# votnhan/VN_celeb_face_recognition

Hardware: AMD Instinct MI355X
Metric: embeddings/sec @ bs=256 (InceptionResnetV1, 160x160) (higher is better)
Workload: dtype bf16

## Files before the change

### vn_celeb_face_recognition_amd/csrc/autotune.cpp

```cpp
#include "engine.h"

#include <algorithm>
#include <cstdio>
#include <cstdlib>
#include <map>

namespace vnf {

EncoderEnv EncoderEnv::read() {
  auto env_int = [](const char* name, int dflt) { const char* v = getenv(name); return v ? atoi(v) : dflt; };
  EncoderEnv e;
  e.fuse = env_int("VNF_FUSE", e.fuse);
  e.direct_stem = env_int("VNF_DIRECT_STEM", e.direct_stem);
  e.stem1a_mfma = env_int("VNF_STEM1A_MFMA", e.stem1a_mfma);
  e.stem_chunk = env_int("VNF_STEM_CHUNK", e.stem_chunk);
  e.ir100_chunk1 = env_int("VNF_IR100_CHUNK1", e.ir100_chunk1);
  e.ir100_chunk2 = env_int("VNF_IR100_CHUNK2", e.ir100_chunk2);
  e.retina_fuse = env_int("VNF_RETINA_FUSE", e.retina_fuse);
  e.ws_persist = env_int("VNF_WS_PERSIST", e.ws_persist);
  e.autotune = env_int("VNF_AUTOTUNE", e.autotune);
  e.force_cfg = env_int("VNF_FORCE_CFG", e.force_cfg);
  e.tune_lanes = env_int("VNF_TUNE_LANES", e.tune_lanes);
  e.autotune_log = env_int("VNF_AUTOTUNE_LOG", e.autotune_log);
  e.tune_final = env_int("VNF_TUNE_FINAL", 1) != 0;
  if (const char* cache = getenv("VNF_TUNE_CACHE")) e.tune_cache = cache;
  return e;
}

int Encoder::autotune() {
  const int enabled = env.autotune, force = env.force_cfg;
  if (!enabled && force < -1) return VNF_OK;
  std::map<std::string, int> cache;
  const char* cache_path = env.tune_cache.empty() ? nullptr : env.tune_cache.c_str();
  bool cache_dirty = false;
  if (cache_path && enabled) {
    if (FILE* f = fopen(cache_path, "r")) {
      char key[256];
      int c;
      while (fscanf(f, "%255s %d", key, &c) == 2) cache[key] = c;
      fclose(f);
    }
  }
  VNF_HIP(hipDeviceSynchronize());
  struct Timers {
    hipEvent_t e0 = nullptr, e1 = nullptr;
    hipStream_t lane_s[4] = {nullptr, nullptr, nullptr, nullptr};
    hipEvent_t lane_e[4] = {nullptr, nullptr, nullptr, nullptr};
    ~Timers() {
      if (e0) (void)hipEventDestroy(e0);
      if (e1) (void)hipEventDestroy(e1);
      for (int l = 0; l < 4; ++l) {
        if (lane_e[l]) (void)hipEventDestroy(lane_e[l]);
// ... 113 lines not shown
```

### vn_celeb_face_recognition_amd/csrc/conv_device.h

```cpp
#pragma once
#include <atomic>

#include "kernels.h"
#include "split_f16.h"

namespace vnf {

typedef __bf16 bf16x8_t __attribute__((ext_vector_type(8)));
typedef _Float16 f16x8_t __attribute__((ext_vector_type(8)));
typedef float f32x4_t __attribute__((ext_vector_type(4)));

struct KArgs {
  const char* x;
  const char* w;
  const float* bias;
  const int4* ktab;
  const char* res;
  const float* slope;
  const char* zero;
  int ldx, H, W, Ho, Wo, sh, sw, ph, pw;
  int K, Kpad, nkt;
  int wrs, wts;
  int ncls, cout_pad;
  int M, Cout, tiles_n, nblk;
// ... 374 lines not shown
          char* const dptr = a.seg_ptr[sg];
          if (a.out_f32)
            store8<float>(dptr + ((size_t)m * a.seg_ld[sg] + (c - a.seg_c0[sg])) * 4, v);
          else
            store8<T>(dptr + ((size_t)m * a.seg_ld[sg] + (c - a.seg_c0[sg])) * ES, v);
        }
      }
      __syncthreads();
    }
  }
}

__device__ __forceinline__ void glds16(const void* gsrc, unsigned lds_base) {
  unsigned keep;
  asm volatile(
      "s_mov_b32 %0, m0\n\ts_mov_b32 m0, %2\n\ts_nop 0\n\tglobal_load_lds_dwordx4 %1, off\n\ts_mov_b32 m0, %0"
      : "=&s"(keep)
      : "v"(gsrc), "s"(lds_base)
      : "memory");
}

template <int N>
__device__ __forceinline__ void wait_dma_and_barrier() {
  asm volatile("s_waitcnt vmcnt(%0) lgkmcnt(0)\n\ts_barrier" ::"n"(N) : "memory");
}

constexpr int patch_epi_bytes(int bm, int bn, int wm) {
  return bm * (bn + 4) * 4 <= 64 * 1024 ? bm * (bn + 4) * 4 : (bm / wm) * (bn + 4) * 4;
}
int patch_num_cfgs();
bool patch_cfg_ok(const ConvArgs& a, int pcfg);
bool patch_cfg_tile(int pcfg, ConvTile& t);
hipError_t launch_patch(const ConvArgs& a, const KArgs& k, int pcfg, hipStream_t s);

int ws_num_cfgs();
bool ws_cfg_ok(const ConvArgs& a, int wcfg);
bool ws_cfg_tile(int wcfg, ConvTile& t);
hipError_t launch_ws(const ConvArgs& a, const KArgs& k, int wcfg, hipStream_t s);

}
```

### vn_celeb_face_recognition_amd/csrc/conv_igemm.hip

```cpp
#include <mutex>
#include <type_traits>
#include <utility>

#include "block35.h"
#include "conv_device.h"

namespace vnf {

template <int AP, int RS>
__device__ __forceinline__ void row_setup(const KArgs& a, int m0, int lrow, int (&abase)[AP], int (&ahi)[AP],
                                          int (&awi)[AP]) {
  const int HoWo = a.Ho * a.Wo;
#pragma unroll
  for (int p = 0; p < AP; ++p) {
    const int m = m0 + lrow + RS * p;
    if (m < a.M) {
      const int n = m / HoWo, r = m - n * HoWo;
      const int ho = r / a.Wo, wo = r - ho * a.Wo;
      ahi[p] = ho * a.sh - a.ph;
      awi[p] = wo * a.sw - a.pw;
      abase[p] = ((n * a.H + ahi[p]) * a.W + awi[p]) * a.ldx;
    } else {
      ahi[p] = -(1 << 24);
      awi[p] = 0;
// ... 264 lines not shown
}

static bool dma_capable(const ConvArgs& a) { return (a.Kpad / (128 / dtype_size(a.dtype))) * 8 * 16 <= 24 * 1024; }

bool conv_cfg_ok(const ConvArgs& a, int cfg) {
  if (cfg >= kNumCfgs + patch_num_cfgs()) return dma_capable(a) && ws_cfg_ok(a, cfg - kNumCfgs - patch_num_cfgs());
  if (cfg >= kNumCfgs) return dma_capable(a) && patch_cfg_ok(a, cfg - kNumCfgs);
  if (cfg < 0) return false;
  const TileCfg& c = kCfgs[cfg];
  if (c.bn > 32 && a.Cout <= c.bn / 2) return false;
  if (((a.Cout + c.bn - 1) / c.bn) * c.bn > a.cout_pad) return false;
  if ((c.bn % 64) && a.Cout % c.bn) return false;
  const int lds = c.s * (c.bm + c.bn) * 128;
  return lds <= 160 * 1024;
}

template <typename T, size_t... I>
static hipError_t launch_cfg(int cfg, const KArgs& k, hipStream_t s, std::index_sequence<I...>) {
  static constexpr hipError_t (*kLaunch[])(const KArgs&, hipStream_t) = {
      launch_dma<T, kCfgs[I].bm, kCfgs[I].bn, kCfgs[I].wm, kCfgs[I].wn, kCfgs[I].s>...};
  return (unsigned)cfg < sizeof...(I) ? kLaunch[cfg](k, s) : hipErrorInvalidValue;
}
template <typename T>
static hipError_t launch_cfg(int cfg, const KArgs& k, hipStream_t s) {
  return launch_cfg<T>(cfg, k, s, std::make_index_sequence<kNumCfgs>{});
}

template <typename T>
static hipError_t launch_typed(const ConvArgs& a, const KArgs& k, hipStream_t s) {
  if (!k.zero) return hipErrorOutOfMemory;
  if (a.cfg >= kNumCfgs + patch_num_cfgs() && conv_cfg_ok(a, a.cfg)) return launch_ws(a, k, a.cfg - kNumCfgs - patch_num_cfgs(), s);
  if (a.cfg >= kNumCfgs && conv_cfg_ok(a, a.cfg)) return launch_patch(a, k, a.cfg - kNumCfgs, s);
  if (a.cfg >= 0 && conv_cfg_ok(a, a.cfg)) return launch_cfg<T>(a.cfg, k, s);
  auto fits = [&](int) { return true; };
  int bn = 128;
  while (bn > 32 && !(fits(bn) && (a.Cout % bn == 0 || a.Cout > 2 * bn))) bn >>= 1;
  if (!fits(bn)) return hipErrorInvalidValue;
  auto blocks = [&](int bm_, int bn_) { return ((a.M + bm_ - 1) / bm_) * ((a.Cout + bn_ - 1) / bn_); };
  while (bn > 64 && blocks(128, bn) < 512) bn >>= 1;
  int bm = 128;
  if (bn <= 64 && blocks(128, bn) < 512) bm = 64;
  const int id = bm == 128 ? (bn == 128 ? 0 : bn == 64 ? 1 : 2) : (bn == 64 ? 3 : 4);
  return launch_cfg<T>(id, k, s);
}

hipError_t launch_conv(const ConvArgs& a, hipStream_t s) {
  if (a.M <= 0) return hipSuccess;
  const int es = dtype_size(a.dtype);
  const int bke = 128 / es;
  if (a.Cout % 8 || a.Kpad % bke || a.nseg < 1 || a.nseg > 4) return hipErrorInvalidValue;
  KArgs k;
  k.x = (const char*)a.x; k.w = (const char*)a.w; k.bias = a.bias; k.ktab = a.ktab;
  k.res = (const char*)a.res; k.slope = a.slope; k.zero = zero_page();
  k.ldx = a.ldx; k.H = a.H; k.W = a.W; k.Ho = a.Ho; k.Wo = a.Wo;
  k.sh = a.sh; k.sw = a.sw; k.ph = a.ph; k.pw = a.pw;
  k.K = a.K; k.Kpad = a.Kpad; k.nkt = a.Kpad / bke;
  k.wrs = a.Kpad * es; k.wts = 128;
  k.ncls = a.ncls; k.cout_pad = a.cout_pad;
  k.M = a.M; k.Cout = a.Cout; k.tiles_n = 0; k.nblk = 0;
  k.ldres = a.ldres; k.act = a.act; k.out_f32 = a.out_f32;
  k.nseg = a.nseg;
  k.KH = a.KH; k.KW = a.KW; k.Cin = a.Cin; k.pp = k.Wp = k.Hv = k.patch_bytes = k.lds_bytes = 0; k.dbg = nullptr;
  for (int i = 0; i < 4; ++i) {
    k.seg_c0[i] = i < a.nseg ? a.seg[i].c0 : 1 << 30;
    k.seg_c1[i] = i < a.nseg ? a.seg[i].c1 : 1 << 30;
    k.seg_ld[i] = i < a.nseg ? a.seg[i].ld : 0;
// ... 14 lines not shown
```

### vn_celeb_face_recognition_amd/csrc/conv_patch.hip

```cpp
#include <map>
#include <mutex>
#include <tuple>
#include <type_traits>
#include <utility>

#include "conv_device.h"
#include "stamp.h"

namespace vnf {

template <typename T, int BM, int BN, int WM, int WN, int S, bool DBG = false>
__global__ __launch_bounds__(WM* WN * 64) void conv_patch_kernel(const KArgs a) {
  extern __shared__ __attribute__((aligned(16))) char smem[];
  constexpr int ES = (int)sizeof(T);
  constexpr int CH = 16 / ES, BKE = 128 / ES;
  constexpr int WTM = BM / WM, WTN = BN / WN, TM = WTM / 16, TN = WTN / 16;
  constexpr int NW = WM * WN, NT = NW * 64, RS = NT / 8;
  constexpr int BPM = (BN + RS - 1) / RS;
  constexpr int STAGE = BN * 128;
  constexpr int EPI = patch_epi_bytes(BM, BN, WM);
  static_assert((NW == 4 || NW == 8) && S >= 3 && BPM <= 8, "4 or 8 waves, ring of >= 3 stages");

  const int tid = threadIdx.x, lane = tid & 63;
  const int wave = __builtin_amdgcn_readfirstlane(tid >> 6);
// ... 172 lines not shown
#pragma unroll
      for (int i = 0; i < TM; ++i)
#pragma unroll
        for (int j = 0; j < TN; ++j) mma_cross(acc[i][j], wh[0][j], wf[1][j], xh[0][i], xf[1][i]);
    } else {
#pragma unroll
      for (int i = 0; i < TM; ++i)
#pragma unroll
        for (int j = 0; j < TN; ++j) mma_cross(acc[i][j], wh[1][j], wf[1][j], xh[1][i], xf[1][i]);
    }
  } else {
    bool pend = false;
    for (int kt = 0; kt < nkt; ++kt) {
      stamp();
      sync_tile(kt);
      stamp();
      read_frags(kt, 0, t0);
      if (pend) mma(1);
      pend = BKE / 2 < a.K - kt * BKE;
      if (pend) read_frags(kt, 1, t1);
      t0 = sP[(kt + 1) * 8 + fgrp];
      t1 = sP[(kt + 1) * 8 + 4 + fgrp];
      mma(0);
    }
    if (pend) mma(1);
  }
  stamp();
  __syncthreads();
  stamp();
  conv_epilogue<T, BM, BN, WM, WN, EPI>(a, acc, smem, m0, n0, a.lds_bytes);
  stamp();
}

struct PatchCfg { int bm, bn, wm, wn, s; };
static constexpr PatchCfg kPatch[] = {
    {256, 32, 8, 1, 3},  {256, 32, 4, 1, 3},  {128, 32, 4, 1, 3},  {256, 64, 4, 2, 3},  {128, 64, 4, 2, 3},
    {128, 64, 2, 2, 3},  {64, 64, 2, 2, 4},   {256, 192, 4, 2, 3}, {128, 192, 2, 4, 3}, {64, 192, 2, 4, 3},
    {128, 256, 2, 4, 3}, {256, 256, 4, 2, 3}, {128, 128, 2, 4, 3}, {256, 128, 4, 2, 3}, {64, 128, 2, 4, 3},
    {64, 128, 2, 2, 4},
    {256, 64, 4, 2, 6},  {128, 64, 4, 2, 6},  {256, 128, 4, 2, 4}, {256, 32, 8, 1, 6},
    {128, 96, 4, 1, 3},  {128, 96, 2, 2, 3},  {64, 192, 1, 4, 3},
    {192, 192, 4, 2, 3},
};
constexpr int kNumPatch = (int)(sizeof(kPatch) / sizeof(kPatch[0]));

int patch_num_cfgs() { return kNumPatch; }
bool patch_cfg_tile(int pcfg, ConvTile& t) {
  if (pcfg < 0 || pcfg >= kNumPatch) return false;
  t = ConvTile{1, kPatch[pcfg].bm, kPatch[pcfg].bn, kPatch[pcfg].wm, kPatch[pcfg].wn, kPatch[pcfg].s};
  return true;
}

static int patch_rows_max(int Wo, int Ho, int KH, int BM) {
  static std::mutex mu;
  static std::map<std::tuple<int, int, int, int>, int> cache;
  std::lock_guard<std::mutex> lk(mu);
  const auto key = std::make_tuple(Wo, Ho, KH, BM);
  auto it = cache.find(key);
  if (it != cache.end()) return it->second;
  int best = 0;
  const long long HoWo = (long long)Ho * Wo;
  for (long long t = 0; t <= HoWo; ++t) {
    const long long m0 = t * BM, m1 = m0 + BM - 1;
    const long long g0 = m0 / Wo, g1 = m1 / Wo;
    const long long v0 = g0 + (g0 / Ho) * (KH - 1), v1 = g1 + (g1 / Ho) * (KH - 1) + KH - 1;
    if (v1 - v0 + 1 > best) best = (int)(v1 - v0 + 1);
  }
  cache[key] = best;
  return best;
}

struct PatchGeom { int pp, Wp, Hv, patch_bytes, lds; };

static bool patch_geom(const ConvArgs& a, const PatchCfg& c, PatchGeom& g) {
  const int es = dtype_size(a.dtype), ch = dtype_chan_align(a.dtype);
  const int planes = a.dtype == F16P ? 2 : 1;
  if (a.sh != 1 || a.sw != 1 || a.Cin % ch || a.Ho != a.H + 2 * a.ph - a.KH + 1 || a.Wo != a.W + 2 * a.pw - a.KW + 1)
    return false;
  g.pp = a.Cin / ch;
  while (g.pp % 4 != 2) ++g.pp;
  g.Wp = a.W + 2 * a.pw;
  g.Hv = a.H + 2 * a.ph;
  const long long slots = (long long)patch_rows_max(a.Wo, a.Ho, a.KH, c.bm) * g.Wp * g.pp;
  if (slots * 16 * planes > 160 * 1024) return false;
  g.patch_bytes = (int)((slots * 16 + 1023) / 1024 * 1024) * planes;
  const int nkt = a.Kpad / (128 / es);
  int lds = c.s * c.bn * 128 + (((nkt + 1) * 8 * 4 + 15) & ~15) + 16 + g.patch_bytes;
  const int epi = patch_epi_bytes(c.bm, c.bn, c.wm);
  if (lds < epi) lds = epi;
  g.lds = lds;
  return lds <= 160 * 1024;
}

bool patch_cfg_ok(const ConvArgs& a, int pcfg) {
  if (pcfg < 0 || pcfg >= kNumPatch) return false;
  const PatchCfg& c = kPatch[pcfg];
  if (a.KH * a.KW == 1) return false;
  if (c.bn > 32 && a.Cout <= c.bn / 2) return false;
  if (((a.Cout + c.bn - 1) / c.bn) * c.bn > a.cout_pad) return false;
  if ((c.bn % 64) && a.Cout % c.bn) return false;
  PatchGeom g;
  return patch_geom(a, c, g);
}

template <typename T, int BM, int BN, int WM, int WN, int S>
static hipError_t launch_one(const KArgs& k, int lds, hipStream_t s) {
  allow_dynamic_lds<conv_patch_kernel<T, BM, BN, WM, WN, S>>(160 * 1024);
  KArgs kk = k;
  const int tiles_m = (k.M + BM - 1) / BM;
  kk.tiles_n = (k.Cout + BN - 1) / BN;
  kk.nblk = tiles_m * kk.tiles_n;
  hipLaunchKernelGGL((conv_patch_kernel<T, BM, BN, WM, WN, S>), dim3(kk.nblk), dim3(WM * WN * 64), lds, s, kk);
  return hipGetLastError();
}

template <typename T, size_t... I>
static hipError_t launch_patch_typed(int pcfg, const KArgs& k, int lds, hipStream_t s, std::index_sequence<I...>) {
  static constexpr hipError_t (*kLaunch[])(const KArgs&, int, hipStream_t) = {
      launch_one<T, kPatch[I].bm, kPatch[I].bn, kPatch[I].wm, kPatch[I].wn, kPatch[I].s>...};
  return (unsigned)pcfg < sizeof...(I) ? kLaunch[pcfg](k, lds, s) : hipErrorInvalidValue;
}
template <typename T>
static hipError_t launch_patch_typed(int pcfg, const KArgs& k, int lds, hipStream_t s) {
  return launch_patch_typed<T>(pcfg, k, lds, s, std::make_index_sequence<kNumPatch>{});
}

#ifdef VNF_STAMPS
constexpr PatchCfg kStamp = {256, 192, 4, 2, 3};
constexpr int patch_cfg_id(const PatchCfg& q) {
  for (int i = 0; i < kNumPatch; ++i)
    if (kPatch[i].bm == q.bm && kPatch[i].bn == q.bn && kPatch[i].wm == q.wm && kPatch[i].wn == q.wn && kPatch[i].s == q.s) return i;
  return -1;
}
constexpr int kStampId = patch_cfg_id(kStamp);
static_assert(kStampId >= 0, "the instrumented tile is one of kPatch");

static hipError_t launch_patch_stamped(const KArgs& k, int lds, hipStream_t s) {
  constexpr auto kernel = conv_patch_kernel<__bf16, kStamp.bm, kStamp.bn, kStamp.wm, kStamp.wn, kStamp.s, true>;
  KArgs kk = k;
  kk.tiles_n = (k.Cout + kStamp.bn - 1) / kStamp.bn;
  kk.nblk = ((k.M + kStamp.bm - 1) / kStamp.bm) * kk.tiles_n;
  return stamped_launch(
      "VNF_PATCH_STAMP", 8 * 40, s,
      [&](long long* dbuf) {
        kk.dbg = dbuf;
        allow_dynamic_lds<kernel>(160 * 1024);
        hipLaunchKernelGGL(kernel, dim3(kk.nblk), dim3(kStamp.wm * kStamp.wn * 64), lds, s, kk);
      },
      [&](FILE* f, const long long* host) {
        fprintf(f, "launch M=%d N=%d nkt=%d nblk=%d\n", k.M, k.Cout, k.nkt, kk.nblk);
        for (int w = 0; w < 8; ++w) {
          fprintf(f, "%d", w);
          for (int i = 0; i < 40; ++i) fprintf(f, " %lld", host[w * 40 + i] ? host[w * 40 + i] - host[0] : -1LL);
          fprintf(f, "\n");
        }
      });
}
#endif

hipError_t launch_patch(const ConvArgs& a, const KArgs& k, int pcfg, hipStream_t s) {
  if (!patch_cfg_ok(a, pcfg) || !k.zero) return hipErrorInvalidValue;
  PatchGeom g;
  patch_geom(a, kPatch[pcfg], g);
  KArgs kk = k;
  kk.KH = a.KH; kk.KW = a.KW; kk.Cin = a.Cin;
  kk.pp = g.pp; kk.Wp = g.Wp; kk.Hv = g.Hv; kk.patch_bytes = g.patch_bytes; kk.lds_bytes = g.lds;
#ifdef VNF_STAMPS
  if (getenv("VNF_PATCH_STAMP") && pcfg == kStampId && a.dtype == BF16 &&
      ((k.M + kStamp.bm - 1) / kStamp.bm) * ((k.Cout + kStamp.bn - 1) / kStamp.bn) > 700)
    return launch_patch_stamped(kk, g.lds, s);
#endif
  switch (a.dtype) {
    case BF16: return launch_patch_typed<__bf16>(pcfg, kk, g.lds, s);
    case F16: return launch_patch_typed<_Float16>(pcfg, kk, g.lds, s);
    case F32: return launch_patch_typed<float>(pcfg, kk, g.lds, s);
    case F16X2: return launch_patch_typed<sf16>(pcfg, kk, g.lds, s);
    case F16P: return launch_patch_typed<pf16>(pcfg, kk, g.lds, s);
  }
  return hipErrorInvalidValue;
}

}
```

### vn_celeb_face_recognition_amd/csrc/conv_ws.hip

```cpp
#include <type_traits>
#include <utility>

#include "conv_device.h"
#include "stamp.h"

namespace vnf {

template <typename T, int BM, int BN, int WM, int WN, int S, int LW, bool DBG = false>
__global__ __launch_bounds__((WM* WN + LW) * 64) void conv_igemm_ws_kernel(const KArgs a) {
  extern __shared__ __attribute__((aligned(16))) char smem[];
  constexpr int ES = (int)sizeof(T);
  constexpr int CH = 16 / ES, BKE = 128 / ES;
  constexpr int WTM = BM / WM, WTN = BN / WN, TM = WTM / 16, TN = WTN / 16;
  constexpr int NC = WM * WN, NT = (NC + LW) * 64;
  constexpr int PA = BM / 8, PB = BN / 8;
  constexpr int LA = PA / LW, LB = PB / LW;
  constexpr int STAGE = (BM + BN) * 128;
  constexpr int CST = BN + 4;
  constexpr int EPI_LDS = (BM * CST * 4 <= S * STAGE && (BM * (BN / 8)) / (NC * 64) <= 8) ? S * STAGE : (BM / WM) * CST * 4;
  constexpr int EPASS = (BM * CST * 4 <= EPI_LDS) ? 1 : WM;
  static_assert(S >= 3 && PA % LW == 0 && PB % LW == 0, "pieces divide over the loader waves");

  const int tid = threadIdx.x, lane = tid & 63;
  const int wave = __builtin_amdgcn_readfirstlane(tid >> 6);
// ... 528 lines not shown
};
constexpr int kNumWs = (int)(sizeof(kWs) / sizeof(kWs[0]));

int ws_num_cfgs() { return kNumWs; }
bool ws_cfg_tile(int wcfg, ConvTile& t) {
  if (wcfg < 0 || wcfg >= kNumWs) return false;
  t = ConvTile{2, kWs[wcfg].bm, kWs[wcfg].bn, kWs[wcfg].wm, kWs[wcfg].wn, kWs[wcfg].s};
  return true;
}

bool ws_cfg_ok(const ConvArgs& a, int wcfg) {
  if (wcfg < 0 || wcfg >= kNumWs) return false;
  const WsCfg& c = kWs[wcfg];
  if (a.Cout <= c.bn / 2) return false;
  if (((a.Cout + c.bn - 1) / c.bn) * c.bn > a.cout_pad) return false;
  if ((c.bn % 64) && a.Cout % c.bn) return false;
  const int lds = c.s * (c.bm + c.bn) * 128 + (a.Kpad / (128 / dtype_size(a.dtype))) * 8 * 16;
  return lds <= 160 * 1024;
}

template <typename T, int BM, int BN, int WM, int WN, int S, int LW>
static hipError_t launch_one_tile(const KArgs& k, hipStream_t s) {
  allow_dynamic_lds<conv_igemm_ws_kernel<T, BM, BN, WM, WN, S, LW>>(160 * 1024);
  KArgs kk = k;
  const int lds = S * (BM + BN) * 128 + k.nkt * 8 * 16;
  const int tiles_m = (k.M + BM - 1) / BM;
  kk.tiles_n = (k.Cout + BN - 1) / BN;
  kk.nblk = tiles_m * kk.tiles_n;
  hipLaunchKernelGGL((conv_igemm_ws_kernel<T, BM, BN, WM, WN, S, LW>), dim3(kk.nblk), dim3((WM * WN + LW) * 64), lds, s,
                     kk);
  return hipGetLastError();
}

static int cu_count() {
  static std::atomic<int> n[16];
  int dev = 0;
  if (hipGetDevice(&dev) != hipSuccess || dev < 0 || dev >= 16) return 256;
  int c = n[dev].load(std::memory_order_relaxed);
  if (c) return c;
  hipDeviceProp_t p;
  if (hipGetDeviceProperties(&p, dev) != hipSuccess) return 256;
  n[dev].store(c = p.multiProcessorCount > 0 ? p.multiProcessorCount : 256, std::memory_order_relaxed);
  return c;
}

static bool ws_persistent(const ConvArgs& a, const KArgs& k) { return a.ws_persist && k.ncls == 1 && !k.out_f32; }

template <typename T, int BM, int BN, int WM, int WN, int S, int LW, bool RES>
static hipError_t launch_persistent(const KArgs& k, hipStream_t s) {
  allow_dynamic_lds<conv_igemm_wsp_kernel<T, BM, BN, WM, WN, S, LW, RES>>(160 * 1024);
  KArgs kk = k;
  const int lds = S * (BM + BN) * 128 + k.nkt * 8 * 16;
  kk.tiles_n = (k.Cout + BN - 1) / BN;
  kk.nblk = ((k.M + BM - 1) / BM) * kk.tiles_n;
  const int per_cu = lds <= 80 * 1024 ? 2 : 1;
  const int slots = cu_count() * per_cu;
  int grid = kk.nblk < slots ? kk.nblk : slots & ~7;
  if (grid < 1) grid = kk.nblk;
  hipLaunchKernelGGL((conv_igemm_wsp_kernel<T, BM, BN, WM, WN, S, LW, RES>), dim3(grid), dim3((WM * WN + LW) * 64), lds, s,
                     kk);
  return hipGetLastError();
}

template <typename T, int BM, int BN, int WM, int WN, int S, int LW>
static hipError_t launch_one(const ConvArgs& a, const KArgs& k, hipStream_t s) {
  if constexpr ((sizeof(T) == 2 || is_planar<T>::value) && (BN / WN / 16) % 2 == 0) {
    if (ws_persistent(a, k)) {
      if (!k.res) return launch_persistent<T, BM, BN, WM, WN, S, LW, false>(k, s);
      if constexpr (sizeof(T) == 2 && (BM / WM / 16) * (BN / WN / 32) <= 8)
        return launch_persistent<T, BM, BN, WM, WN, S, LW, true>(k, s);
    }
  }
  return launch_one_tile<T, BM, BN, WM, WN, S, LW>(k, s);
}

template <typename T, size_t... I>
static hipError_t launch_ws_typed(int wcfg, const ConvArgs& a, const KArgs& k, hipStream_t s, std::index_sequence<I...>) {
  static constexpr hipError_t (*kLaunch[])(const ConvArgs&, const KArgs&, hipStream_t) = {
      launch_one<T, kWs[I].bm, kWs[I].bn, kWs[I].wm, kWs[I].wn, kWs[I].s, kWs[I].lw>...};
  return (unsigned)wcfg < sizeof...(I) ? kLaunch[wcfg](a, k, s) : hipErrorInvalidValue;
}
template <typename T>
static hipError_t launch_ws_typed(int wcfg, const ConvArgs& a, const KArgs& k, hipStream_t s) {
  return launch_ws_typed<T>(wcfg, a, k, s, std::make_index_sequence<kNumWs>{});
}

#ifdef VNF_STAMPS
constexpr WsCfg kStamp = {128, 192, 2, 2, 3, 4};
constexpr int ws_cfg_id(const WsCfg& q) {
// ... 50 lines not shown
```

### vn_celeb_face_recognition_amd/csrc/engine.cpp

```cpp
#include "engine.h"
#include "split_f16.h"

#include <cstdio>
#include <cstring>

namespace vnf {

static thread_local std::string g_err;
void set_error(const std::string& msg) { g_err = msg; }
int fail(int code, const std::string& msg) {
  g_err = msg;
  return code;
}
const char* last_error_cstr() { return g_err.c_str(); }

HandleBase::~HandleBase() {
  for (void* p : allocs) (void)hipFree(p);
}
void* HandleBase::dalloc(size_t bytes) {
  void* p = nullptr;
  if (bytes == 0) bytes = 16;
  hipError_t e = hipMalloc(&p, bytes);
  if (e != hipSuccess) {
    set_error(std::string("hipMalloc: ") + hipGetErrorString(e));
// ... 64 lines not shown
int Encoder::add_buf(int H, int W, int C) {
  bufs.push_back(Buf{H, W, C});
  return (int)bufs.size() - 1;
}

ConvArgs Encoder::conv_args(const ConvLayer& L, int n0, int nn) const {
  const int es = dtype_size(dtype);
  ConvArgs a;
  memset(&a, 0, sizeof(a));
  a.dtype = dtype;
  a.x = at(L.x_buf, n0, L.x_coff);
  a.ldx = bufs[L.x_buf].C; a.H = L.H; a.W = L.W; a.Cin = L.cin; a.Ho = L.Ho; a.Wo = L.Wo;
  a.KH = L.KH; a.KW = L.KW; a.sh = L.sh; a.sw = L.sw; a.ph = L.ph; a.pw = L.pw;
  a.w = L.w; a.K = L.K; a.Kpad = L.Kpad; a.bias = L.bias; a.ncls = L.ncls; a.cout_pad = L.cout_pad;
  a.ktab = L.ktab; a.M = nn * L.Ho * L.Wo; a.Cout = L.cout; a.nseg = L.nseg;
  for (int i = 0; i < L.nseg; ++i) {
    a.seg[i].c0 = L.seg[i].c0; a.seg[i].c1 = L.seg[i].c1;
    if (L.seg[i].buf == -2) {
      a.seg[i].ptr = emb_raw + (size_t)n0 * emb_ld;
      a.seg[i].ld = emb_ld;
    } else {
      const Buf& ob = bufs[L.seg[i].buf];
      a.seg[i].ptr = ob.ptr + ((size_t)n0 * ob.elems_per_image() + L.seg[i].coff) * (L.out_f32 ? 4 : es);
      a.seg[i].ld = ob.C;
    }
  }
  if (L.res_buf >= 0) {
    a.res = at(L.res_buf, n0, L.res_coff);
    a.ldres = bufs[L.res_buf].C;
  }
  a.act = L.act; a.slope = L.slope; a.out_f32 = L.out_f32;
  a.cfg = L.cfg;
  a.ws_persist = env.ws_persist;
  return a;
}

int Encoder::finalize() {
  const int es = dtype_size(dtype);
  for (auto& b : bufs) {
    const size_t bytes = b.elems_per_image() * es * (size_t)max_batch;
    b.ptr = (char*)dalloc(bytes);
    if (!b.ptr) return VNF_E_HIP;
    VNF_HIP(hipMemset(b.ptr, 0, bytes));
  }
  emb_raw = (float*)dalloc((size_t)max_batch * emb_ld * 4);
  if (!emb_raw) return VNF_E_HIP;
  macs_alg = macs_exec = 0;
  for (auto& c : convs) { macs_alg += c.macs_alg; macs_exec += c.macs_exec; }
  if (groups.empty()) groups.push_back({0, (int)ops.size(), 1 << 30});
  const int rc = prepare_fused();
  if (rc != VNF_OK) return rc;
  fused_at.assign(ops.size(), -1);
  for (size_t i = 0; i < fused.size(); ++i)
    if (fused[i].active) fused_at[fused[i].first] = (int)i;
  tune_dirty = true;
  return VNF_OK;
}

Encoder::~Encoder() {
  for (int i = 0; i < 4; ++i) {
    if (join_ev[i]) (void)hipEventDestroy(join_ev[i]);
    if (side[i]) (void)hipStreamDestroy(side[i]);
  }
  if (fork_ev) (void)hipEventDestroy(fork_ev);
  for (hipEvent_t ev : ctx_ev)
    if (ev) (void)hipEventDestroy(ev);
// ... 259 lines not shown
```

### vn_celeb_face_recognition_amd/csrc/engine.h

```cpp
#pragma once
#include <hip/hip_runtime.h>
#include <stdint.h>

#include <string>
#include <unordered_map>
#include <vector>

#include "../../include/vnface.h"
#include "kernels.h"

namespace vnf {

void set_error(const std::string& msg);
int fail(int code, const std::string& msg);
const char* last_error_cstr();

#define VNF_HIP(expr)                                                                         \
  do {                                                                                        \
    hipError_t _e = (expr);                                                                   \
    if (_e != hipSuccess)                                                                     \
      return ::vnf::fail(VNF_E_HIP, std::string(#expr) + ": " + hipGetErrorString(_e));       \
  } while (0)

enum class HandleKind { Encoder = 1, Mlp, Mtcnn, MlpTrainer, Retina, HeadTrainer, ConvProbe, Gallery };
// ... 98 lines not shown
  std::string name;
};

struct SeLayer {
  std::string name;
  int C, part_buf;
  float *w1 = nullptr, *b1 = nullptr, *w2 = nullptr, *b2 = nullptr;
  float slope_se = 0.f, slope_out = 0.f;
};

struct Group { int first, last, chunk; };

struct FusedStack {
  enum class Kind { StemMid, Block35, Block17, Block8 } kind = Kind::Block17;
  std::string label;
  int first = 0, last = 0;
  int in_buf = -1, out_buf = -1;
  int nblocks = 0;
  int conv0 = 0;
  void* wstream = nullptr;
  float* bias = nullptr;
  void* wtail = nullptr;
  bool active = false;
  bool stack = false;
  double macs_alg = 0;
  int ext_last = 0, ext_conv = -1, ext_out_buf = -1;
  bool ext = false;
  int end() const { return ext ? ext_last : last; }
};

struct Tap { int buf, coff, C; };

struct EncoderEnv {
  int fuse = 95, direct_stem = 1, stem1a_mfma = 2, retina_fuse = 3, ws_persist = 1;
  int stem_chunk = 0, ir100_chunk1 = 0, ir100_chunk2 = 0;
  int autotune = 1, force_cfg = -2, tune_lanes = 0, autotune_log = 0;
  bool tune_final = true;
  std::string tune_cache;
  static EncoderEnv read();
};

struct RunExtra {
  float* out2 = nullptr;
  const uint8_t* prep_src = nullptr;
  int prep_s = 0;
};

constexpr int ARCH_MLP = -1, ARCH_RNET = -2, ARCH_ONET = -3, ARCH_RETINA = -5;

struct Encoder : HandleBase {
  static constexpr HandleKind KIND = HandleKind::Encoder;
  Encoder() : HandleBase(KIND) {}
  ~Encoder() override;
  int arch, dtype, max_batch, in_size;
  std::vector<Buf> bufs;
  std::vector<ConvLayer> convs;
  std::vector<DwLayer> dws;
  std::vector<DwPwLayer> dwpws;
  std::vector<SeLayer> ses;
  float *rstem_wa = nullptr, *rstem_bias = nullptr;
  std::vector<Op> ops;
  std::vector<Group> groups;
  std::vector<FusedStack> fused;
  std::vector<int> fused_at;
  int prepare_fused();
  int launch_fused(const FusedStack& f, int n0, int nn, hipStream_t s);
  std::unordered_map<std::string, Tap> taps;
// ... 52 lines not shown
```

### vn_celeb_face_recognition_amd/csrc/kernels.h

```cpp
#pragma once
#include <hip/hip_runtime.h>
#include <stdint.h>

#include "../../include/vnface.h"

namespace vnf {

enum DType { F32 = 0, BF16 = 1, F16 = 2, F16X2 = 5, F16P = 6 };
inline int dtype_size(int dt) { return (dt == F32 || dt == F16X2 || dt == F16P) ? 4 : 2; }
inline int dtype_chan_align(int dt) { return dt == F16P ? 8 : 16 / dtype_size(dt); }

enum Act { ACT_NONE = 0, ACT_RELU = 1, ACT_PRELU = 2 };

struct ConvSeg {
  int c0, c1;
  void* ptr;
  int ld;
};

struct ConvArgs {
  int dtype;
  const void* x;
  int ldx;
  int H, W, Cin;
  int Ho, Wo;
  int KH, KW, sh, sw, ph, pw;
  const void* w;
  int K, Kpad;
  const float* bias;
  int ncls;
  int cout_pad;
  const int4* ktab;
  int M, Cout;
  int nseg;
  ConvSeg seg[4];
  const void* res;
  int ldres;
  int act;
  const float* slope;
  int out_f32;
  int cfg;
  int ws_persist;
};

hipError_t launch_conv(const ConvArgs& a, hipStream_t s);
int conv_num_cfgs();
bool conv_cfg_ok(const ConvArgs& a, int cfg);
void conv_family_sizes(int sizes[3]);
struct ConvTile { int family, bm, bn, wm, wn, stages; };
bool conv_cfg_tile(int cfg, ConvTile& t);

hipError_t launch_pack_input(const void* x, int x_dtype, void* out, int dtype, int n, int hw, hipStream_t s);

hipError_t launch_stem_conv1a(const void* x, int x_dtype, void* y, int ldy, int dtype, int n, const float* wt, int mode,
                              hipStream_t s);

struct PoolWindow { int k, pad; bool ceil; };
inline int pool_out_size(int in, PoolWindow w) {
  const int span = in + 2 * w.pad - w.k;
  return span < 0 && !w.ceil ? 0 : (span + (w.ceil ? 1 : 0)) / 2 + 1;
}
hipError_t launch_maxpool(const void* x, int ldx, void* y, int ldy, int dtype, int n, int H, int W, int C, PoolWindow w,
                          hipStream_t s);

hipError_t launch_emotion_prep(const uint8_t* faces, int n, int S, void* out, int out_dtype, bool packed, hipStream_t s);

hipError_t launch_augment_faces(const uint8_t* faces, int n_faces, int S, const int32_t* index, const vnf_aug_param* params, int n,
                                int T, void* x_out, int out_dtype, uint8_t* u8_out, hipStream_t s);

hipError_t launch_softmax_topk(const float* logits, int n, int C, int k, int32_t* idx, float* prob, hipStream_t s);

hipError_t launch_copy_rows_f32(const float* src, int lds, float* dst, int ldd, int n, int C, hipStream_t s);

hipError_t launch_avgpool(const void* x, int ldx, void* y, int dtype, int n, int HW, int C, hipStream_t s);

// ... 25 lines not shown
```

Measured before the change: 279,700.

## Add persistent warp-specialized patch conv kernel with DMA loader waves

```diff
diff --git a/vn_celeb_face_recognition_amd/csrc/autotune.cpp b/vn_celeb_face_recognition_amd/csrc/autotune.cpp
--- a/vn_celeb_face_recognition_amd/csrc/autotune.cpp
+++ b/vn_celeb_face_recognition_amd/csrc/autotune.cpp
@@ -18,6 +18,7 @@
   e.ir100_chunk2 = env_int("VNF_IR100_CHUNK2", e.ir100_chunk2);
   e.retina_fuse = env_int("VNF_RETINA_FUSE", e.retina_fuse);
   e.ws_persist = env_int("VNF_WS_PERSIST", e.ws_persist);
+  e.patch_persist = env_int("VNF_PATCH_PERSIST", e.patch_persist);
   e.autotune = env_int("VNF_AUTOTUNE", e.autotune);
   e.force_cfg = env_int("VNF_FORCE_CFG", e.force_cfg);
   e.tune_lanes = env_int("VNF_TUNE_LANES", e.tune_lanes);
diff --git a/vn_celeb_face_recognition_amd/csrc/conv_device.h b/vn_celeb_face_recognition_amd/csrc/conv_device.h
--- a/vn_celeb_face_recognition_amd/csrc/conv_device.h
+++ b/vn_celeb_face_recognition_amd/csrc/conv_device.h
@@ -430,10 +430,12 @@
 bool patch_cfg_ok(const ConvArgs& a, int pcfg);
 bool patch_cfg_tile(int pcfg, ConvTile& t);
 hipError_t launch_patch(const ConvArgs& a, const KArgs& k, int pcfg, hipStream_t s);
+int patch_heuristic_cfg(const ConvArgs& a);
 
 int ws_num_cfgs();
 bool ws_cfg_ok(const ConvArgs& a, int wcfg);
 bool ws_cfg_tile(int wcfg, ConvTile& t);
 hipError_t launch_ws(const ConvArgs& a, const KArgs& k, int wcfg, hipStream_t s);
-
-}
+int conv_cu_count();
+
+}
diff --git a/vn_celeb_face_recognition_amd/csrc/conv_igemm.hip b/vn_celeb_face_recognition_amd/csrc/conv_igemm.hip
--- a/vn_celeb_face_recognition_amd/csrc/conv_igemm.hip
+++ b/vn_celeb_face_recognition_amd/csrc/conv_igemm.hip
@@ -320,6 +320,7 @@
   if (a.cfg >= kNumCfgs + patch_num_cfgs() && conv_cfg_ok(a, a.cfg)) return launch_ws(a, k, a.cfg - kNumCfgs - patch_num_cfgs(), s);
   if (a.cfg >= kNumCfgs && conv_cfg_ok(a, a.cfg)) return launch_patch(a, k, a.cfg - kNumCfgs, s);
   if (a.cfg >= 0 && conv_cfg_ok(a, a.cfg)) return launch_cfg<T>(a.cfg, k, s);
+  if (const int pc = patch_heuristic_cfg(a); pc >= 0 && dma_capable(a)) return launch_patch(a, k, pc, s);
   auto fits = [&](int) { return true; };
   int bn = 128;
   while (bn > 32 && !(fits(bn) && (a.Cout % bn == 0 || a.Cout > 2 * bn))) bn >>= 1;
diff --git a/vn_celeb_face_recognition_amd/csrc/conv_patch.hip b/vn_celeb_face_recognition_amd/csrc/conv_patch.hip
--- a/vn_celeb_face_recognition_amd/csrc/conv_patch.hip
+++ b/vn_celeb_face_recognition_amd/csrc/conv_patch.hip
@@ -228,7 +228,234 @@
   stamp();
 }
 
-struct PatchCfg { int bm, bn, wm, wn, s; };
+template <typename T, int BM, int BN, int WM, int WN, int S, int LW>
+__global__ __launch_bounds__((WM* WN + LW) * 64) void conv_patch_wsp_kernel(const KArgs a) {
+  static_assert(sizeof(T) == 2, "register epilogue: 2-byte elements");
+  extern __shared__ __attribute__((aligned(16))) char smem[];
+  constexpr int ES = (int)sizeof(T);
+  constexpr int CH = 16 / ES, BKE = 128 / ES;
+  constexpr int WTM = BM / WM, WTN = BN / WN, TM = WTM / 16, TN = WTN / 16;
+  constexpr int NC = WM * WN, NT = (NC + LW) * 64;
+  constexpr int PB = BN / 8, LB = PB / LW;
+  constexpr int STAGE = BN * 128;
+  static_assert(S >= 3 && PB % LW == 0 && TN % 2 == 0 && BM % (WM * 16) == 0 && BN % (WN * 16) == 0, "tile shape");
+
+  const int tid = threadIdx.x, lane = tid & 63;
+  const int wave = __builtin_amdgcn_readfirstlane(tid >> 6);
+  const int nkt = a.nkt;
+  const int G = (int)gridDim.x;
+  const int ntile = (a.nblk - (int)blockIdx.x + G - 1) / G;
+  const int Q = ntile * nkt;
+
+  const int ptab_bytes = ((nkt + 1) * 8 * 4 + 15) & ~15;
+  int* sP = reinterpret_cast<int*>(smem + S * STAGE);
+  char* const zslot = smem + S * STAGE + ptab_bytes;
+  const char* const patch = zslot + 16;
+  for (int i = tid; i < nkt * 8; i += NT) {
+    const int4 e = a.ktab[i];
+    const int cc = (e.x - (e.y * a.W + e.z) * a.ldx) / CH;
+    sP[i] = e.w ? ((e.y * a.Wp + e.z) * a.pp + cc) * 16 : -1;
+  }
+  if (tid < 4) reinterpret_cast<int*>(zslot)[tid] = 0;
+  __syncthreads();
+
+  auto tile_at = [&](int it, int& m0, int& n0, int& m_last) {
+    const int bid = xcd_remap((int)blockIdx.x + it * G, a.nblk);
+    const int tile_m = bid / a.tiles_n, tile_n = bid - tile_m * a.tiles_n;
+    m0 = tile_m * BM;
+    n0 = tile_n * BN;
+    m_last = min(m0 + BM, a.M) - 1;
+  };
+
+  if (wave >= NC) {
+    const int lw = wave - NC;
+    const int prow = lane >> 3, lcol = lane & 7;
+    const int lchunk = lcol ^ prow;
+    const unsigned lds0 = (unsigned)reinterpret_cast<uintptr_t>((__attribute__((address_space(3))) char*)smem);
+    const unsigned lds_patch = lds0 + (unsigned)(S * STAGE + ptab_bytes + 16);
+    const float inv_pp = 1.f / (float)a.pp, inv_wp = 1.f / (float)a.Wp, inv_hv = 1.f / (float)a.Hv;
+    auto quot = [](int s, int d, float inv) {
+      int q = (int)((float)s * inv);
+      const int r = s - q * d;
+      if (r >= d) ++q;
+      if (r < 0) --q;
+      return q;
+    };
+    const int cpb = a.Cin / CH;
+    auto issue_patch = [&](int it) {
+      int m0, n0, m_last;
+      tile_at(it, m0, n0, m_last);
+      const int g0 = m0 / a.Wo, g1 = m_last / a.Wo;
+      const int v0 = g0 + (g0 / a.Ho) * (a.KH - 1);
+      const int v1 = g1 + (g1 / a.Ho) * (a.KH - 1) + a.KH - 1;
+      const int nslots = (v1 - v0 + 1) * a.Wp * a.pp;
+      const int npieces = (nslots + 63) >> 6;
+      for (int pc = lw; pc < npieces; pc += LW) {
+        const int s = pc * 64 + lane;
+        const char* src = a.zero;
+        if (s < nslots) {
+          const int p = quot(s, a.pp, inv_pp), c = s - p * a.pp;
+          const int py = quot(p, a.Wp, inv_wp), px = p - py * a.Wp;
+          const int v = v0 + py, n = quot(v, a.Hv, inv_hv);
+          const int iy = v - n * a.Hv - a.ph, ix = px - a.pw;
+          if (c < cpb && (unsigned)iy < (unsigned)a.H && (unsigned)ix < (unsigned)a.W)
+            src = a.x + ((size_t)((n * a.H + iy) * a.W + ix) * a.ldx) * ES + c * 16;
+        }
+        glds16(src, __builtin_amdgcn_readfirstlane(lds_patch + (unsigned)pc * 1024u));
+      }
+    };
+    const char* wsrc = nullptr;
+    auto setup_w = [&](int it) {
+      int m0, n0, m_last;
+      tile_at(it, m0, n0, m_last);
+      wsrc = a.w + (size_t)(n0 + lw * 8 + prow) * a.wrs + lchunk * 16;
+    };
+    int it_i = 0, kt_i = 0, st_i = 0;
+    auto issue_w = [&]() {
+      const unsigned sbase = __builtin_amdgcn_readfirstlane(lds0 + (unsigned)(st_i * STAGE) + (unsigned)(lw * 1024));
+#pragma unroll
+      for (int p = 0; p < LB; ++p)
+        glds16(wsrc + (size_t)(p * LW * 8) * a.wrs + (size_t)kt_i * a.wts, sbase + p * (LW * 1024));
+      st_i = st_i + 1 == S ? 0 : st_i + 1;
+      if (++kt_i == nkt) {
+        kt_i = 0;
+        if (++it_i < ntile) setup_w(it_i);
+      }
+    };
+    setup_w(0);
+    issue_patch(0);
+#pragma unroll
+    for (int t = 0; t < S - 1; ++t)
+      if (t < Q) issue_w();
+    int q = 0;
+    for (int it = 0; it < ntile; ++it) {
+      for (int kt = 0; kt < nkt; ++kt, ++q) {
+        if (kt != 0 && q + S - 2 < Q)
+          wait_dma_and_barrier<(S - 2) * LB>();
+        else
+          wait_dma_and_barrier<0>();
+        if (q + S - 1 < Q) issue_w();
+      }
+      asm volatile("s_barrier" ::: "memory");
+      if (it + 1 < ntile) issue_patch(it + 1);
+    }
+    return;
+  }
+
+  const int wm = wave / WN, wn = wave % WN;
+  const int frow = lane & 15, fgrp = lane >> 4;
+  typedef T tx4 __attribute__((ext_vector_type(4)));
+  const bool relu = a.act == ACT_RELU, prelu = a.act == ACT_PRELU;
+  int st = 0;
+  for (int it = 0; it < ntile; ++it) {
+    int m0, n0, m_last;
+    tile_at(it, m0, n0, m_last);
+    const int g0 = m0 / a.Wo;
+    const int v0 = g0 + (g0 / a.Ho) * (a.KH - 1);
+    int pb[TM];
+#pragma unroll
+    for (int i = 0; i < TM; ++i) {
+      const int m = min(m0 + wm * WTM + i * 16 + frow, m_last);
+      const int g = m / a.Wo, ox = m - g * a.Wo;
+      const int vb = g + (g / a.Ho) * (a.KH - 1);
+      pb[i] = ((vb - v0) * a.Wp + ox) * a.pp * 16;
+    }
+    f32x4_t acc[TM][TN];
+#pragma unroll
+    for (int i = 0; i < TM; ++i)
+#pragma unroll
+      for (int j = 0; j < TN; ++j) acc[i][j] = f32x4_t{0.f, 0.f, 0.f, 0.f};
+    uint4 xf[TM], wf[TN];
+    auto read_frags = [&](int ks, int t) {
+      const char* sB = smem + st * STAGE;
+#pragma unroll
+      for (int i = 0; i < TM; ++i) xf[i] = *reinterpret_cast<const uint4*>(patch + (t >= 0 ? pb[i] + t : -16));
+#pragma unroll
+      for (int j = 0; j < TN; ++j) {
+        const int row = wn * WTN + j * 16 + frow;
+        wf[j] = *reinterpret_cast<const uint4*>(sB + row * 128 + (((ks * 4 + fgrp) ^ (row & 7)) << 4));
+      }
+    };
+    auto mma = [&]() {
+#pragma unroll
+      for (int i = 0; i < TM; ++i)
+#pragma unroll
+        for (int j = 0; j < TN; ++j) mma_chunk<T>(acc[i][j], wf[j], xf[i]);
+    };
+    auto join = [&]() {
+      asm volatile("s_waitcnt lgkmcnt(0)\n\ts_barrier" ::: "memory");
+    };
+    int t0 = sP[fgrp], t1 = sP[4 + fgrp];
+    for (int kt = 0; kt < nkt; ++kt) {
+      const bool last = kt + 1 == nkt;
+      const bool two = BKE / 2 < a.K - kt * BKE;
+      const int ktn = last ? 0 : kt + 1;
+      join();
+      read_frags(0, t0);
+      t0 = sP[ktn * 8 + fgrp];
+      if (last && !two) join();
+      mma();
+      if (two) {
+        read_frags(1, t1);
+        if (last) join();
+        mma();
+      }
+      t1 = sP[ktn * 8 + 4 + fgrp];
+      st = st + 1 == S ? 0 : st + 1;
+    }
+
+#pragma unroll
+    for (int j = 0; j < TN; j += 2) {
+      const int cq = n0 + wn * WTN + j * 16 + fgrp * 4;
+      const f32x4_t b0 = cq < a.Cout ? *reinterpret_cast<const f32x4_t*>(a.bias + cq) : f32x4_t{0.f, 0.f, 0.f, 0.f};
+      const f32x4_t b1 =
+          cq + 16 < a.Cout ? *reinterpret_cast<const f32x4_t*>(a.bias + cq + 16) : f32x4_t{0.f, 0.f, 0.f, 0.f};
+      f32x4_t s0 = {0.f, 0.f, 0.f, 0.f}, s1 = s0;
+      if (prelu) {
+        if (cq < a.Cout) s0 = *reinterpret_cast<const f32x4_t*>(a.slope + cq);
+        if (cq + 16 < a.Cout) s1 = *reinterpret_cast<const f32x4_t*>(a.slope + cq + 16);
+      }
+      const int c = n0 + wn * WTN + (j + (fgrp & 1)) * 16 + (fgrp >> 1) * 8;
+      int sg = 0;
+#pragma unroll
+      for (int s2 = 1; s2 < 4; ++s2)
+        if (s2 < a.nseg && c >= a.seg_c0[s2]) sg = s2;
+      char* const dcol = a.seg_ptr[sg] + (size_t)(c - a.seg_c0[sg]) * ES;
+      const int dld = a.seg_ld[sg];
+#pragma unroll
+      for (int i = 0; i < TM; ++i) {
+        float v0[4], v1[4];
+#pragma unroll
+        for (int e = 0; e < 4; ++e) {
+          v0[e] = acc[i][j][e] + b0[e];
+          v1[e] = acc[i][j + 1][e] + b1[e];
+        }
+        if (relu) {
+#pragma unroll
+          for (int e = 0; e < 4; ++e) { v0[e] = fmaxf(v0[e], 0.f); v1[e] = fmaxf(v1[e], 0.f); }
+        }
+        if (prelu) {
+#pragma unroll
+          for (int e = 0; e < 4; ++e) {
+            v0[e] = v0[e] > 0.f ? v0[e] : v0[e] * s0[e];
+            v1[e] = v1[e] > 0.f ? v1[e] : v1[e] * s1[e];
+          }
+        }
+        const int m = m0 + wm * WTM + i * 16 + frow;
+        tx4 o0, o1;
+#pragma unroll
+        for (int e = 0; e < 4; ++e) { o0[e] = (T)v0[e]; o1[e] = (T)v1[e]; }
+        const uint2 p0 = __builtin_bit_cast(uint2, o0), p1 = __builtin_bit_cast(uint2, o1);
+        const auto sx = __builtin_amdgcn_permlane16_swap(p0.x, p1.x, false, false);
+        const auto sy = __builtin_amdgcn_permlane16_swap(p0.y, p1.y, false, false);
+        if (m < a.M && c < a.Cout)
+          *reinterpret_cast<uint4*>(dcol + (size_t)m * dld * ES) = uint4{sx[0], sy[0], sx[1], sy[1]};
+      }
+    }
+  }
+}
+
+struct PatchCfg { int bm, bn, wm, wn, s, lw; };
 static constexpr PatchCfg kPatch[] = {
     {256, 32, 8, 1, 3},  {256, 32, 4, 1, 3},  {128, 32, 4, 1, 3},  {256, 64, 4, 2, 3},  {128, 64, 4, 2, 3},
     {128, 64, 2, 2, 3},  {64, 64, 2, 2, 4},   {256, 192, 4, 2, 3}, {128, 192, 2, 4, 3}, {64, 192, 2, 4, 3},
@@ -237,6 +464,7 @@
     {256, 64, 4, 2, 6},  {128, 64, 4, 2, 6},  {256, 128, 4, 2, 4}, {256, 32, 8, 1, 6},
     {128, 96, 4, 1, 3},  {128, 96, 2, 2, 3},  {64, 192, 1, 4, 3},
     {192, 192, 4, 2, 3},
+    {224, 192, 2, 2, 3, 4},
 };
 constexpr int kNumPatch = (int)(sizeof(kPatch) / sizeof(kPatch[0]));
 
@@ -299,26 +527,51 @@
   return patch_geom(a, c, g);
 }
 
-template <typename T, int BM, int BN, int WM, int WN, int S>
-static hipError_t launch_one(const KArgs& k, int lds, hipStream_t s) {
-  allow_dynamic_lds<conv_patch_kernel<T, BM, BN, WM, WN, S>>(160 * 1024);
+static bool patch_persistent(const ConvArgs& a) {
+  return a.patch_persist && a.ncls == 1 && !a.out_f32 && !a.res && (a.dtype == BF16 || a.dtype == F16) &&
+         (long long)(a.M / (a.Ho * a.Wo) + 1) * (a.H + 2 * a.ph) < (1 << 22);
+}
+
+int patch_heuristic_cfg(const ConvArgs& a) {
+  if (!patch_persistent(a)) return -1;
+  for (int i = 0; i < kNumPatch; ++i)
+    if (kPatch[i].lw > 0 && a.Cout == kPatch[i].bn && patch_cfg_ok(a, i)) return i;
+  return -1;
+}
+
+template <typename T, int BM, int BN, int WM, int WN, int S, int LW>
+static hipError_t launch_one(const ConvArgs& a, const KArgs& k, int lds, hipStream_t s) {
   KArgs kk = k;
   const int tiles_m = (k.M + BM - 1) / BM;
   kk.tiles_n = (k.Cout + BN - 1) / BN;
   kk.nblk = tiles_m * kk.tiles_n;
-  hipLaunchKernelGGL((conv_patch_kernel<T, BM, BN, WM, WN, S>), dim3(kk.nblk), dim3(WM * WN * 64), lds, s, kk);
+  if constexpr (LW > 0 && sizeof(T) == 2) {
+    if (patch_persistent(a)) {
+      allow_dynamic_lds<conv_patch_wsp_kernel<T, BM, BN, WM, WN, S, LW>>(160 * 1024);
+      const int slots = conv_cu_count();
+      int grid = kk.nblk < slots ? kk.nblk : slots & ~7;
+      if (grid < 1) grid = kk.nblk;
+      hipLaunchKernelGGL((conv_patch_wsp_kernel<T, BM, BN, WM, WN, S, LW>), dim3(grid), dim3((WM * WN + LW) * 64), lds, s,
+                         kk);
+      return hipGetLastError();
+    }
+  }
+  constexpr int WN1 = (LW > 0 && is_planar<T>::value) ? 2 * WN : WN;
+  allow_dynamic_lds<conv_patch_kernel<T, BM, BN, WM, WN1, S>>(160 * 1024);
+  hipLaunchKernelGGL((conv_patch_kernel<T, BM, BN, WM, WN1, S>), dim3(kk.nblk), dim3(WM * WN1 * 64), lds, s, kk);
   return hipGetLastError();
 }
 
 template <typename T, size_t... I>
-static hipError_t launch_patch_typed(int pcfg, const KArgs& k, int lds, hipStream_t s, std::index_sequence<I...>) {
-  static constexpr hipError_t (*kLaunch[])(const KArgs&, int, hipStream_t) = {
-      launch_one<T, kPatch[I].bm, kPatch[I].bn, kPatch[I].wm, kPatch[I].wn, kPatch[I].s>...};
-  return (unsigned)pcfg < sizeof...(I) ? kLaunch[pcfg](k, lds, s) : hipErrorInvalidValue;
+static hipError_t launch_patch_typed(int pcfg, const ConvArgs& a, const KArgs& k, int lds, hipStream_t s,
+                                     std::index_sequence<I...>) {
+  static constexpr hipError_t (*kLaunch[])(const ConvArgs&, const KArgs&, int, hipStream_t) = {
+      launch_one<T, kPatch[I].bm, kPatch[I].bn, kPatch[I].wm, kPatch[I].wn, kPatch[I].s, kPatch[I].lw>...};
+  return (unsigned)pcfg < sizeof...(I) ? kLaunch[pcfg](a, k, lds, s) : hipErrorInvalidValue;
 }
 template <typename T>
-static hipError_t launch_patch_typed(int pcfg, const KArgs& k, int lds, hipStream_t s) {
-  return launch_patch_typed<T>(pcfg, k, lds, s, std::make_index_sequence<kNumPatch>{});
+static hipError_t launch_patch_typed(int pcfg, const ConvArgs& a, const KArgs& k, int lds, hipStream_t s) {
+  return launch_patch_typed<T>(pcfg, a, k, lds, s, std::make_index_sequence<kNumPatch>{});
 }
 
 #ifdef VNF_STAMPS
@@ -367,11 +620,11 @@
     return launch_patch_stamped(kk, g.lds, s);
 #endif
   switch (a.dtype) {
-    case BF16: return launch_patch_typed<__bf16>(pcfg, kk, g.lds, s);
-    case F16: return launch_patch_typed<_Float16>(pcfg, kk, g.lds, s);
-    case F32: return launch_patch_typed<float>(pcfg, kk, g.lds, s);
-    case F16X2: return launch_patch_typed<sf16>(pcfg, kk, g.lds, s);
-    case F16P: return launch_patch_typed<pf16>(pcfg, kk, g.lds, s);
+    case BF16: return launch_patch_typed<__bf16>(pcfg, a, kk, g.lds, s);
+    case F16: return launch_patch_typed<_Float16>(pcfg, a, kk, g.lds, s);
+    case F32: return launch_patch_typed<float>(pcfg, a, kk, g.lds, s);
+    case F16X2: return launch_patch_typed<sf16>(pcfg, a, kk, g.lds, s);
+    case F16P: return launch_patch_typed<pf16>(pcfg, a, kk, g.lds, s);
   }
   return hipErrorInvalidValue;
 }
diff --git a/vn_celeb_face_recognition_amd/csrc/conv_ws.hip b/vn_celeb_face_recognition_amd/csrc/conv_ws.hip
--- a/vn_celeb_face_recognition_amd/csrc/conv_ws.hip
+++ b/vn_celeb_face_recognition_amd/csrc/conv_ws.hip
@@ -584,7 +584,7 @@
   return hipGetLastError();
 }
 
-static int cu_count() {
+int conv_cu_count() {
   static std::atomic<int> n[16];
   int dev = 0;
   if (hipGetDevice(&dev) != hipSuccess || dev < 0 || dev >= 16) return 256;
@@ -606,7 +606,7 @@
   kk.tiles_n = (k.Cout + BN - 1) / BN;
   kk.nblk = ((k.M + BM - 1) / BM) * kk.tiles_n;
   const int per_cu = lds <= 80 * 1024 ? 2 : 1;
-  const int slots = cu_count() * per_cu;
+  const int slots = conv_cu_count() * per_cu;
   int grid = kk.nblk < slots ? kk.nblk : slots & ~7;
   if (grid < 1) grid = kk.nblk;
   hipLaunchKernelGGL((conv_igemm_wsp_kernel<T, BM, BN, WM, WN, S, LW, RES>), dim3(grid), dim3((WM * WN + LW) * 64), lds, s,
diff --git a/vn_celeb_face_recognition_amd/csrc/engine.cpp b/vn_celeb_face_recognition_amd/csrc/engine.cpp
--- a/vn_celeb_face_recognition_amd/csrc/engine.cpp
+++ b/vn_celeb_face_recognition_amd/csrc/engine.cpp
@@ -120,6 +120,7 @@
   a.act = L.act; a.slope = L.slope; a.out_f32 = L.out_f32;
   a.cfg = L.cfg;
   a.ws_persist = env.ws_persist;
+  a.patch_persist = env.patch_persist;
   return a;
 }
 
diff --git a/vn_celeb_face_recognition_amd/csrc/engine.h b/vn_celeb_face_recognition_amd/csrc/engine.h
--- a/vn_celeb_face_recognition_amd/csrc/engine.h
+++ b/vn_celeb_face_recognition_amd/csrc/engine.h
@@ -154,7 +154,7 @@
 struct Tap { int buf, coff, C; };
 
 struct EncoderEnv {
-  int fuse = 95, direct_stem = 1, stem1a_mfma = 2, retina_fuse = 3, ws_persist = 1;
+  int fuse = 95, direct_stem = 1, stem1a_mfma = 2, retina_fuse = 3, ws_persist = 1, patch_persist = 1;
   int stem_chunk = 0, ir100_chunk1 = 0, ir100_chunk2 = 0;
   int autotune = 1, force_cfg = -2, tune_lanes = 0, autotune_log = 0;
   bool tune_final = true;
diff --git a/vn_celeb_face_recognition_amd/csrc/kernels.h b/vn_celeb_face_recognition_amd/csrc/kernels.h
--- a/vn_celeb_face_recognition_amd/csrc/kernels.h
+++ b/vn_celeb_face_recognition_amd/csrc/kernels.h
@@ -41,6 +41,7 @@
   int out_f32;
   int cfg;
   int ws_persist;
+  int patch_persist;
 };
 
 hipError_t launch_conv(const ConvArgs& a, hipStream_t s);
```

Result: no change. 280,100, median of 6 (+0.1%).
